# Kinetica-jl/Kinetica.jl

Measured on AMD Instinct MI355X. Metric: RHS evals/sec (batched sweep) + wall-clock per solve_network, 10k-species CRN, higher is better.
Workload: dtype f64; 1 GPU; synthetic CRN 10000 species / 50000 reactions (seed 12345), batched RHS sweep, B=4096 states per GPU with per-state Arrhenius k (500-1200 K); states_per_gpu=4096, parallelism=replicas x1 (no data-path collective)

## Files before the change

include/kinetica_hip.h:

```cpp
#ifndef KINETICA_HIP_H
#define KINETICA_HIP_H

#include <stdint.h>

#ifdef __cplusplus
extern "C" {
#endif

enum {
  KIN_OK = 0,
  KIN_ERR_INVALID_ARG = 1,
  KIN_ERR_UNSUPPORTED = 2,
  KIN_ERR_DEVICE = 3,
  KIN_ERR_SOLVE_FAILED = 4,
  KIN_ERR_CAPACITY = 5,
  KIN_ERR_STATE = 6
};

enum {
  KIN_RETCODE_SUCCESS = 0,
  KIN_RETCODE_MAXITERS = 1,
  KIN_RETCODE_DTLESSTHANMIN = 2,
  KIN_RETCODE_UNSTABLE = 3
};

typedef struct kin_network kin_network;

int kin_network_create(int64_t n_species, int64_t n_reactions,
                       const int64_t* reac_ptr, const int64_t* reac_idx, const int64_t* reac_sto,
                       const int64_t* prod_ptr, const int64_t* prod_idx, const int64_t* prod_sto,
                       int index_base, kin_network** out);
int kin_network_destroy(kin_network* h);
int kin_network_sizes(const kin_network* h, int64_t* n_species, int64_t* n_reactions);
const char* kin_last_error(const kin_network* h);

int kin_set_rates(kin_network* h, const double* k);
int kin_get_rates(kin_network* h, double* k_out);
int kin_set_arrhenius(kin_network* h, const double* Ea, const double* A, double k_max, double t_mult);
int kin_rates_at(kin_network* h, double T, double* k_out);
int kin_arrhenius_eval(const double* Ea, const double* A, int64_t n, double k_max, double t_mult,
                       double T, double* k_out);
int kin_rate_table(kin_network* h, const double* T, int64_t n_stops, double* out_table);

int kin_rhs(kin_network* h, const double* u, double* du);
int kin_rhs_batched(kin_network* h, int64_t B, const double* u, const double* k, double* du);
int kin_rhs_batched_dev(kin_network* h, int64_t B, const double* d_u, const double* d_k, double* d_du, void* stream);

int kin_lib_layout(kin_network* h, int index_base, int64_t* k_len, int64_t* species_of_lib, int64_t* slot_of_reaction,
                   int32_t* species_identity, int64_t* info);
int kin_lib_layout_host(int64_t n_species, int64_t n_reactions, const int64_t* reac_ptr, const int64_t* reac_idx,
                        const int64_t* reac_sto, const int64_t* prod_ptr, const int64_t* prod_idx, const int64_t* prod_sto,
                        int index_base, int hubs, int64_t* info, int64_t* species_of_lib, int64_t* slot_of_reaction,
                        uint64_t* rec, int32_t* rowtab, int32_t* seg_q, int32_t* win_off, int32_t* win_cnt, int32_t* copy_src,
                        int32_t* seg_k);
int kin_lu_analyze_host(int64_t n_species, int64_t n_reactions, const int64_t* reac_ptr, const int64_t* reac_idx,
                        const int64_t* reac_sto, const int64_t* prod_ptr, const int64_t* prod_idx, const int64_t* prod_sto,
                        int index_base, int hub_degree, int max_rounds, int max_tail_degree, int max_degree, int min_round,
                        int64_t* info);
int kin_states_to_lib_dev(kin_network* h, int64_t B, const double* d_in, double* d_out, void* stream);
int kin_states_from_lib_dev(kin_network* h, int64_t B, const double* d_in, double* d_out, void* stream);
int kin_rates_to_lib_dev(kin_network* h, int64_t B, const double* d_k, double* d_k_lib, void* stream);
int kin_rate_table_lib_dev(kin_network* h, const double* T, int64_t n_stops, double* d_out);
int kin_rhs_tiled_dev(kin_network* h, int64_t B, const double* d_u_lib, const double* d_k_lib, const double* d_T,
                      double* d_du_lib, void* stream);
int kin_rhs_batched_T_dev(kin_network* h, int64_t B, const double* d_u, const double* d_T, double* d_du, void* stream);
int kin_rhs_batched_klib_dev(kin_network* h, int64_t B, const double* d_u, const double* d_k_lib, double* d_du, void* stream);

int kin_flux_batched_dev(kin_network* h, int64_t B, const double* d_u, const double* d_k, const int64_t* d_k_row, const double* d_T,
                         const double* d_w, double* d_flux, double* d_rates, void* stream);
int kin_flux_batched(kin_network* h, int64_t B, const double* u, const double* k, int64_t n_k_rows, const int64_t* k_row,
                     const double* T, const double* w, double* flux, double* rates);
int kin_solution_flux(kin_network* h, const double* w, const double* k, int64_t n_k_rows, const int64_t* k_row,
                      const double* T_rows, double* flux, double* rates);

int kin_jac_nnz(kin_network* h, int64_t* nnz);
int kin_jac_pattern(kin_network* h, int64_t* rowptr, int64_t* colidx, int index_base);
int kin_jac_values(kin_network* h, const double* u, double* vals);

typedef struct kin_params {
  double tspan0, tspan1;
  double abstol;
  double reltol;
  int32_t adaptive_tols;
  int32_t update_tols;
  int32_t solve_chunks;
  int32_t ban_negatives;
  double solve_chunkstep;
// ... 79 lines not shown
```

kinetica_jl_amd/capi.py:

```python
from __future__ import annotations

import ctypes
import os
from ctypes import POINTER, c_char_p, c_double, c_int, c_int32, c_int64, c_void_p

import numpy as np

_HERE = os.path.dirname(os.path.abspath(__file__))
LIB_PATH = os.environ.get("KIN_LIB_PATH", os.path.join(_HERE, "libkinetica_hip.so"))

KIN_OK, KIN_ERR_INVALID_ARG, KIN_ERR_UNSUPPORTED, KIN_ERR_DEVICE, KIN_ERR_SOLVE_FAILED, KIN_ERR_CAPACITY, KIN_ERR_STATE = range(7)
RETCODE_NAMES = {0: "Success", 1: "MaxIters", 2: "DtLessThanMin", 3: "Unstable"}

SYMBOLS = [
    "kin_network_create", "kin_network_destroy", "kin_network_sizes", "kin_last_error",
    "kin_set_rates", "kin_get_rates", "kin_set_arrhenius", "kin_rates_at", "kin_arrhenius_eval",
    "kin_rate_table", "kin_rhs", "kin_rhs_batched", "kin_rhs_batched_dev",
    "kin_jac_nnz", "kin_jac_pattern", "kin_jac_values", "kin_solve", "kin_solve_explicit", "kin_solve_continuous", "kin_solution_size",
    "kin_solution_copy", "kin_solution_max", "kin_integrator_init", "kin_integrator_init_continuous", "kin_integrator_step",
    "kin_integrator_state",
    "kin_newton_solve", "kin_device_count", "kin_set_device", "kin_version", "kin_solution_dot", "kin_rate_table_rows",
    "kin_solution_max_dev", "kin_rate_table_dev", "kin_rhs_block_dev",
    "kin_lib_layout", "kin_lib_layout_host", "kin_states_to_lib_dev", "kin_states_from_lib_dev", "kin_rates_to_lib_dev", "kin_rate_table_lib_dev",
    "kin_rhs_tiled_dev", "kin_rhs_batched_T_dev", "kin_rhs_batched_klib_dev", "kin_abi_version", "kin_struct_size",
    "kin_solve_ensemble", "kin_lu_analyze_host", "kin_solve_ensemble_continuous", "kin_solve_ensemble_discrete",
    "kin_resident_probe", "kin_newton_probe", "kin_step_probe",
    "kin_flux_batched", "kin_flux_batched_dev", "kin_solution_flux",
]
ABI_VERSION = 6


STEP_ROWS, STEP_CTRL, STEP_IARGS, STEP_DARGS = 28, 18, 12, 24
STEP_ROW = dict(D=0, y=8, psi=9, d=10, scale=11, f0=12, f1=13, ytmp=14, cs=15, K=16, x=23, out=24, y_new=25, u=26, b=27)
STEP_CTRL_FIELDS = ("dy_norm_old", "dy_norm", "err_norm", "err_m_norm", "err_p_norm", "crate", "scratch0", "scratch1", "scratch2",
                    "scratch3", "newton_done", "converged", "n_iter", "nonfinite", "any_negative", "ticket", "lu_bad", "spec_go")
STEP_OPS = dict(init_D=0, predict=1, accept=2, accept_predict=3, change_D=4, interp=5, norms=6, newton=7, rk_combine=8, rk_error=9, vec=10)
STEP_VEC_OPS = dict(load_u0=0, cs_from_y=1, y_from_cs_clipped=2, y_from_d0=3, ytmp_from_d0=4, ytmp_axpy=5, save_y=6, interp=7)
STEP_IARG_NAMES = ("member", "order", "aux", "copy_out", "go", "iter", "maxit", "publish_always", "crate_from_ctrl", "ban_negatives", "seq")
STEP_DARG_NAMES = ("atol", "rtol", "h", "upd", "tol", "rate_max", "crate0", "tol_first", "dy_first_max", "c", "ts", "t", "h_abs")
STEP_DARG_W = 13


class KinParams(ctypes.Structure):
    _fields_ = [("tspan0", c_double), ("tspan1", c_double), ("abstol", c_double), ("reltol", c_double),
                ("adaptive_tols", c_int32), ("update_tols", c_int32), ("solve_chunks", c_int32),
                ("ban_negatives", c_int32), ("solve_chunkstep", c_double), ("maxiters", c_int64),
                ("save_interval", c_double), ("dtmin", c_double)]


class KinStats(ctypes.Structure):
    _fields_ = [(n, c_int64) for n in ("n_steps", "n_rejected", "n_rhs", "n_jac", "n_factor", "n_linsolve",
                                        "n_newton_fail", "n_chunks", "n_restarts", "n_retries")] + \
               [("final_abstol", c_double), ("final_reltol", c_double), ("wall_seconds", c_double)] + \
               [(n, c_int64) for n in ("lu_dense_dim", "lu_sparse_rows", "lu_rounds", "lu_nnz", "n_lu_reused", "lu_slots", "n_bad_pivot", "n_lu_dropped")]

    def as_dict(self):
        return {n: getattr(self, n) for n, _ in self._fields_}


class KineticaHipError(RuntimeError):
# ... 102 lines not shown


def device_count():
    n = c_int(0)
    lib().kin_device_count(ctypes.byref(n))
    return n.value


def lib_layout_host(net, hubs=0):
    L = lib()
    arrs = [np.ascontiguousarray(a, dtype=np.int64) for a in (net.reac_ptr, net.reac_idx, net.reac_sto, net.prod_ptr,
                                                              net.prod_idx, net.prod_sto)]
    P32, PU64 = POINTER(c_int32), POINTER(ctypes.c_uint64)
    L.kin_lib_layout_host.argtypes = [c_int64, c_int64] + [POINTER(c_int64)] * 6 + [c_int, c_int, POINTER(c_int64), POINTER(c_int64),
                                                                                  POINTER(c_int64), PU64, P32, P32, P32, P32, P32, P32]
    info = np.zeros(10, np.int64)
    head = [int(net.n_species), int(net.n_reactions)] + [_p64(a) for a in arrs] + [0, int(hubs), _p64(info)]
    st = L.kin_lib_layout_host(*head, None, None, None, None, None, None, None, None, None)
    if st != KIN_OK:
        raise KineticaHipError(st, "network has no tiled layout")
    h, T, P, E, n_copy, BS, wbase, Q, k_len, has_singles = [int(x) for x in info]
    sp = np.empty(net.n_species, np.int64); slot = np.empty(net.n_reactions, np.int64)
    rec = np.empty(max(P, 1), np.uint64); rowtab = np.empty(max(2 * Q, 1), np.int32); seg_q = np.empty(T + 1, np.int32)
    woff = np.empty(T, np.int32); wcnt = np.empty(T, np.int32); copy_src = np.empty(max(n_copy, 1), np.int32)
    seg_k = np.empty(2 * T, np.int32)
    i32 = lambda a: a.ctypes.data_as(P32)
    st = L.kin_lib_layout_host(*head, _p64(sp), _p64(slot), rec.ctypes.data_as(PU64), i32(rowtab), i32(seg_q), i32(woff), i32(wcnt),
                               i32(copy_src), i32(seg_k))
    assert st == KIN_OK
    return dict(k_len=k_len, has_singles=bool(has_singles), seg_k=seg_k.reshape(T, 2), h=h, T=T, P=P, E=E, n_copy=n_copy, BS=BS, wbase=wbase, Q=Q, species_of_lib=sp, slot_of_reaction=slot,
                rec=rec[:P], rowtab=rowtab[:2 * Q].reshape(Q, 2), seg_q=seg_q, win_off=woff, win_cnt=wcnt, copy_src=copy_src[:n_copy])


def lu_analyze_host(net, hub_degree=0, max_rounds=0, max_tail_degree=0, max_degree=0, min_round=0):
    L = lib()
    arrs = [np.ascontiguousarray(a, dtype=np.int64) for a in (net.reac_ptr, net.reac_idx, net.reac_sto, net.prod_ptr,
                                                              net.prod_idx, net.prod_sto)]
    L.kin_lu_analyze_host.argtypes = [c_int64, c_int64] + [POINTER(c_int64)] * 6 + [c_int] * 6 + [POINTER(c_int64)]
    info = np.zeros(12, np.int64)
    st = L.kin_lu_analyze_host(int(net.n_species), int(net.n_reactions), *[_p64(a) for a in arrs], 0, int(hub_degree), int(max_rounds),
                               int(max_tail_degree), int(max_degree), int(min_round), _p64(info))
    if st != KIN_OK:
        raise KineticaHipError(st, "symbolic LU analysis failed")
    keys = ("ns", "m", "rounds", "nnzU", "nnzZ", "nnzV", "nnzLZ", "nnzNVU", "w_size", "fused_products", "plan_entries", "plan_tasks")
    return {k: int(v) for k, v in zip(keys, info)}


def arrhenius_eval(Ea, A, T, k_max=None, t_mult=1.0):
    Ea, A = _f64(Ea), _f64(A)
    out = np.empty(len(Ea))
    st = lib().kin_arrhenius_eval(_pd(Ea), _pd(A), len(Ea), float("nan") if k_max is None else k_max, t_mult, T, _pd(out))
    if st != KIN_OK:
        raise KineticaHipError(st, lib().kin_last_error(None).decode())
    return out


class HipNetwork:

    def __init__(self, n_species, reac_ptr, reac_idx, reac_sto, prod_ptr, prod_idx, prod_sto, index_base=0):
        arrs = [np.ascontiguousarray(a, dtype=np.int64) for a in (reac_ptr, reac_idx, reac_sto, prod_ptr, prod_idx, prod_sto)]
        self._h = c_void_p()
        st = lib().kin_network_create(int(n_species), len(arrs[0]) - 1, *[_p64(a) for a in arrs], index_base,
                                      ctypes.byref(self._h))
        if st != KIN_OK:
            raise KineticaHipError(st, lib().kin_last_error(None).decode())
        self.n = int(n_species)
# ... 388 lines not shown
```

kinetica_jl_amd/csrc/network.cpp:

```cpp
#include "network.hpp"

#include <algorithm>
#include <map>
#include <numeric>
#include <string>

namespace kin {

SegPlanHost build_seg_plan(int64_t n_rows, const int32_t* ptr, const int32_t* dst, const int32_t* a,
                           const int32_t* b, const float* c, bool skip_empty, const int32_t* aux,
                           std::vector<int32_t>* slot_of_entry) {
  SegPlanHost P;
  const bool prod = b != nullptr;
  if (slot_of_entry) slot_of_entry->assign((size_t)ptr[n_rows], -1);
  std::vector<int32_t> shorts, longs;
  for (int64_t i = 0; i < n_rows; i++) {
    int32_t len = ptr[i + 1] - ptr[i];
    if (len == 0 && skip_empty) continue;
    (len <= SegPlanHost::SHORT_MAX ? shorts : longs).push_back((int32_t)i);
  }
  {
    std::vector<size_t> start(SegPlanHost::SHORT_MAX + 2, 0);
    for (int32_t r : shorts) start[ptr[r + 1] - ptr[r] + 1]++;
    for (size_t l = 1; l < start.size(); l++) start[l] += start[l - 1];
    std::vector<int32_t> ordered(shorts.size());
    for (int32_t r : shorts) ordered[start[ptr[r + 1] - ptr[r]]++] = r;
    shorts.swap(ordered);
  }
  const size_t n_groups = (shorts.size() + 63) / 64;
  P.grp_off.reserve(n_groups + 1);
  P.grp_off.push_back(0);
  for (size_t g0 = 0; g0 < shorts.size(); g0 += 64) {
    const size_t g1 = std::min(shorts.size(), g0 + 64);
    P.grp_off.push_back(P.grp_off.back() + (ptr[shorts[g1 - 1] + 1] - ptr[shorts[g1 - 1]]));
  }
  {
    const size_t ell = (size_t)P.grp_off.back() * 64;
    if (a) P.ell_a.assign(ell, 0);
    if (b) P.ell_b.assign(ell, prod ? -1 : 0);
    if (!prod) P.ell_c.assign(ell, 0.0f);
// ... 139 lines not shown
      return kq;
    };
    std::map<Key, std::vector<int32_t>> waiting;
    std::vector<int32_t> partner(R, -1);
    std::vector<char> is_plain(R, 0);
    for (int64_t r = 0; r < R; r++) {
      bool plain;
      Key fwd = key_of(r, +1, plain);
      is_plain[r] = plain;
      if (!plain) continue;
      Key rev = key_of(r, -1, plain);
      auto it = waiting.find(rev);
      if (it != waiting.end() && !it->second.empty()) {
        int32_t q = it->second.back(); it->second.pop_back();
        partner[r] = q; partner[q] = (int32_t)r;
      } else waiting[fwd].push_back((int32_t)r);
    }
    for (int64_t r = 0; r < R; r++) {
      if (partner[r] >= 0 && partner[r] < r) continue;
      H.pair_rec.push_back(s16(H.slot_sp[4 * r + 0]) | (s16(H.slot_sp[4 * r + 1]) << 16));
      H.pair_rec.push_back(s16(H.slot_sp[4 * r + 2]) | (s16(H.slot_sp[4 * r + 3]) << 16));
      H.pair_rec.push_back((uint32_t)H.slot_co[r]);
      H.pair_rec.push_back(is_plain[r] ? 0xffffffffu : (s16(H.x0[r]) | (s16(H.x1[r]) << 16)));
      H.pair_k.push_back((int32_t)r);
      H.pair_k.push_back(partner[r]);
    }
    H.pairs_adjacent = (R % 2 == 0) && (H.n_pairs() * 2 == R);
    for (int64_t p = 0; p < H.n_pairs() && H.pairs_adjacent; p++)
      if (H.pair_k[2 * p] != 2 * p || H.pair_k[2 * p + 1] != 2 * p + 1) H.pairs_adjacent = false;
    H.pairs_block = !H.pairs_adjacent && (H.n_pairs() * 2 == R) && R > 0;
    for (int64_t p = 0; p < H.n_pairs() && H.pairs_block; p++)
      if (H.pair_k[2 * p] != p || H.pair_k[2 * p + 1] != H.n_pairs() + p) H.pairs_block = false;
    if ((H.pairs_adjacent || H.pairs_block) && N + 64 <= 16384) {
      bool ok = true;
      std::vector<int32_t> inst((size_t)4 * H.n_pairs());
      for (int64_t p = 0; p < H.n_pairs() && ok; p++) {
        const uint32_t s01 = H.pair_rec[4 * p], s23 = H.pair_rec[4 * p + 1], co = H.pair_rec[4 * p + 2];
        const uint32_t sl[4] = {s01 & 0xffffu, s01 >> 16, s23 & 0xffffu, s23 >> 16};
        uint64_t side[2][2];
        int cnt[2] = {0, 0};
        for (int j = 0; j < 4 && ok; j++) {
          if (sl[j] == 0xffffu) continue;
          const int c = (int)(int8_t)(co >> (8 * j));
          if (c == 0 || c < -2 || c > 2) { ok = false; break; }
          const int sd = c < 0 ? 0 : 1;
          for (int q = 0; q < (c < 0 ? -c : c); q++) {
            if (cnt[sd] >= 2) { ok = false; break; }
            side[sd][cnt[sd]++] = sl[j];
          }
        }
        if (!ok) break;
        const uint64_t dummy = (uint64_t)N + (uint64_t)(p & 63);
        for (int sd = 0; sd < 2; sd++)
          while (cnt[sd] < 2) side[sd][cnt[sd]++] = dummy;
        for (int j = 0; j < 4; j++) inst[4 * p + j] = (int32_t)side[j / 2][j % 2];
      }
      if (ok) {
        const int64_t P = H.n_pairs();
        const int64_t spare = (160 * 1024) / 16 - (N + 64);
        const int K = (int)std::max<int64_t>(0, std::min<int64_t>(32, spare / 7));
        std::vector<int64_t> refs(N, 0);
        for (int64_t q = 0; q < 4 * P; q++) if (inst[q] < N) refs[inst[q]]++;
        std::vector<int32_t> order(N);
        std::iota(order.begin(), order.end(), 0);
        std::stable_sort(order.begin(), order.end(), [&](int32_t x, int32_t y) { return refs[x] > refs[y]; });
        std::vector<int32_t> rank_of(N, -1);
        H.sweep_copy_species.clear();
        for (int r = 0; r < K && r < N && refs[order[r]] >= 64; r++) {
          rank_of[order[r]] = r;
          for (int c = 1; c < 8; c++) H.sweep_copy_species.push_back(order[r]);
        }
        for (int64_t p = 0; p < P; p++) {
          uint64_t f[4];
          for (int j = 0; j < 4; j++) {
            const int32_t sp = inst[4 * p + j];
            const int c = (int)(p & 7);
            f[j] = (sp < N && rank_of[sp] >= 0 && c > 0) ? (uint64_t)(N + 64 + rank_of[sp] * 7 + (c - 1)) : (uint64_t)sp;
          }
          const uint64_t w = f[0] | (f[1] << 14) | (f[2] << 28) | (f[3] << 42);
          H.pair_rec64.push_back((uint32_t)w);
          H.pair_rec64.push_back((uint32_t)(w >> 32));
        }
        for (int64_t p = P; P > 0 && p < P + SWEEP_REC_PAD; p++) {
          const uint64_t d = (uint64_t)N + (uint64_t)(p & 63);
          const uint64_t w = d | (d << 14) | (d << 28) | (d << 42);
          H.pair_rec64.push_back((uint32_t)w);
          H.pair_rec64.push_back((uint32_t)(w >> 32));
        }
      }
    }
    if (!H.pairs_adjacent && !H.pairs_block && (size_t)(N + 64) * 16 <= 160 * 1024) {
      const int64_t P = H.n_pairs();
      for (int64_t p = 0; p < P; p++) {
        const uint32_t s01 = H.pair_rec[4 * p], s23 = H.pair_rec[4 * p + 1], co = H.pair_rec[4 * p + 2], ops = H.pair_rec[4 * p + 3];
        const uint32_t sl[4] = {s01 & 0xffffu, s01 >> 16, s23 & 0xffffu, s23 >> 16};
        const uint32_t dummy = (uint32_t)N + (uint32_t)(p & 63);
        uint32_t side[2][2] = {{dummy, dummy}, {dummy, dummy}};
        int cnt[2] = {0, 0};
        if (ops == 0xffffffffu) {
          for (int j = 0; j < 4; j++) {
            if (sl[j] == 0xffffu) continue;
            const int c = (int)(int8_t)(co >> (8 * j));
            const int sd = c < 0 ? 0 : 1;
            for (int q = 0; q < (c < 0 ? -c : c) && cnt[sd] < 2; q++) side[sd][cnt[sd]++] = sl[j];
          }
        } else {
          H.gen_expl.push_back((int32_t)p);
        }
        H.gen_rec8.push_back(side[0][0] | (side[0][1] << 16));
        H.gen_rec8.push_back(side[1][0] | (side[1][1] << 16));
      }
      H.gen_k = H.pair_k;
// ... 108 lines not shown
```

kinetica_jl_amd/csrc/network.hpp:

```cpp
#pragma once
#include <cstdint>
#include <vector>

#include "common.hpp"

namespace kin {

struct SegPlanHost {
  static constexpr int SHORT_MAX = 8;
  static constexpr int SEG_LEN = 256;
  static constexpr int BLK_PASS = 12288;
  std::vector<int32_t> grp_off;
  std::vector<int32_t> grp_dst;
  std::vector<int32_t> grp_aux;
  std::vector<int32_t> ell_a, ell_b;
  std::vector<float> ell_c;
  std::vector<int32_t> seg_beg, seg_end;
  std::vector<int32_t> seg_dst;
  std::vector<int32_t> seg_aux;
  std::vector<int32_t> blk_beg, blk_end, blk_dst, blk_aux;
  std::vector<int32_t> long_a, long_b;
  std::vector<float> long_c;
  int32_t val_base = -1;
  int32_t ell_total = 0, long_total = 0;
// ... 11 lines not shown
struct NetworkHost {
  int64_t N = 0, R = 0;
  std::vector<int32_t> x0, x1;
  std::vector<int32_t> y0, y1;
  bool products_le2 = true;
  std::vector<int32_t> slot_sp;
  std::vector<int32_t> slot_co;
  std::vector<uint32_t> pair_rec;
  std::vector<int32_t> pair_k;
  std::vector<uint32_t> gen_rec8;
  std::vector<int32_t> gen_k;
  std::vector<int32_t> gen_expl;
  std::vector<int32_t> sweep_copy_species;
  std::vector<uint32_t> pair_rec64;
  int32_t big_H = 0;
  bool big_tail_by_species = false;
  std::vector<int32_t> big_spec_of_label;
  std::vector<uint32_t> big_rec;
  std::vector<uint32_t> big_rec8;
  std::vector<int32_t> big_expl;
  std::vector<int32_t> big_tail_ptr;
  std::vector<uint32_t> big_tail_ent;
  bool pairs_adjacent = false;
  bool pairs_block = false;
  int64_t n_pairs() const { return (int64_t)pair_k.size() / 2; }
  std::vector<int32_t> sp_ptr, sp_rxn;
  std::vector<float> sp_coef;
  std::vector<int32_t> j_ptr, j_col, j_diag;
  std::vector<int32_t> jc_ptr, jc_src;
  std::vector<float> jc_coef;
  int64_t nnz() const { return (int64_t)j_col.size(); }
};

NetworkHost compile_network(int64_t n_species, int64_t n_reactions, const int64_t* reac_ptr,
                            const int64_t* reac_idx, const int64_t* reac_sto, const int64_t* prod_ptr,
                            const int64_t* prod_idx, const int64_t* prod_sto, int index_base);

}
```

kinetica_jl_amd/csrc/tiled.cpp:

```cpp
#include "tiled.hpp"

#include <algorithm>
#include <array>
#include <map>
#include <chrono>
#include <cstdio>
#include <cstdlib>
#include <numeric>

namespace kin {

namespace {

struct UnionFind {
  std::vector<int32_t> par;
  explicit UnionFind(int32_t n) : par(n) { std::iota(par.begin(), par.end(), 0); }
  int32_t find(int32_t x) {
    while (par[x] != x) { par[x] = par[par[x]]; x = par[x]; }
    return x;
  }
  void unite(int32_t a, int32_t b) {
    a = find(a); b = find(b);
    if (a != b) par[b] = a;
  }
};

struct Rec { int32_t f[4]; int32_t kf, kr; };


struct SegCtx {
  const std::vector<Rec>& recs;
  const std::vector<int64_t>& cnt;
  const std::vector<int32_t>& lib_of_species;
// ... 26 lines not shown
  const int32_t n = (int32_t)sorted.size(), h = cx.h;
  Placement pl;
  pl.order = sorted; pl.labs.resize(n); pl.flipped.assign(n, 0);
  for (int32_t i = 0; i < n; i++)
    for (int j = 0; j < 4; j++) {
      uint64_t opt[1 + TILED_COPIES];
      const int no = label_options(cx, sorted[i], j, opt);
      pl.labs[i][j] = no == 0 ? (uint64_t)(h + (i & (TILED_DUMMY - 1))) : opt[no > 1 ? (i & 7) : 0];
    }
  return pl;
}

Placement place_bank_aware(const SegCtx& cx, const std::vector<int32_t>& sorted) {
  const std::vector<Rec>& recs = cx.recs;
  const std::vector<int64_t>& cnt = cx.cnt;
  const int32_t n = (int32_t)sorted.size(), h = cx.h;
  const int SCAN = cx.scan;
  const bool chunked = cx.chunked;
  Placement pl;
  pl.order.resize(n); pl.labs.resize(n); pl.flipped.assign(n, 0);
  std::vector<int32_t>& placed = pl.order;
  std::vector<std::array<uint64_t, 4>>& labs = pl.labs;
  std::vector<char>& flipped = pl.flipped;
  int64_t& sched_slots = pl.slots; int64_t& sched_conflicts = pl.conflicts; int64_t& dbg_defer = pl.deferred;
  auto cls = [&](int32_t p) { return cls_of(recs[p]); };
  auto kind = [&](int32_t p) { return kind_of(cx, recs[p]); };
  auto options = [&](int32_t p, int j, uint64_t* opt) { return label_options(cx, p, j, opt); };
  struct Cand { int32_t p; uint16_t m16[4]; uint32_t m32[4]; int64_t hard; bool sides; int cls; };
  auto make_cand = [&](int32_t p) {
    Cand c{p, {0, 0, 0, 0}, {0, 0, 0, 0}, 0, false, cls(p)};
    for (int j = 0; j < 4; j++) {
      uint64_t opt[1 + TILED_COPIES];
      const int no = options(p, j, opt);
      for (int o = 0; o < no; o++) { c.m16[j] |= (uint16_t)(1u << (opt[o] & 15)); c.m32[j] |= 1u << (opt[o] & 31); }
      if (no > 0) c.hard = std::max(c.hard, cnt[recs[p].f[j]]);
    }
    c.sides = recs[p].kr >= 0 && (recs[p].f[1] >= 0) == (recs[p].f[3] >= 0);
    return c;
  };
  auto sources = [](int o, int* src) {
    const int s0 = (o & 4) ? 2 : 0, s1 = (o & 4) ? 0 : 2;
    src[0] = s0 + (o & 1); src[1] = s0 + ((o & 1) ^ 1);
    src[2] = s1 + ((o >> 1) & 1); src[3] = s1 + (((o >> 1) & 1) ^ 1);
  };
  bool present[8] = {false, false, false, false, false, false, false, false};
  for (int32_t x = 0; x < n; x++) present[kind(sorted[x]) | cls(sorted[x])] = true;
  auto later_home = [&](int x, int c, int kd) {
    for (int c2 = c + 1; c2 < 4; c2++) if (present[kd | c2] && (x & ~c2) == 0) return true;
    return false;
  };
  std::vector<Cand> deferred;
  uint32_t used[4] = {0, 0, 0, 0}, used32[4] = {0, 0, 0, 0};
  int32_t i = 0;
  for (int32_t a = 0; a < n;) {
    int32_t b = a;
    const int c_run = cls(sorted[a]), k_run = kind(sorted[a]);
    while (b < n && cls(sorted[b]) == c_run && kind(sorted[b]) == k_run) b++;
    const bool live[4] = {true, (c_run & 1) != 0, true, (c_run & 2) != 0};
    std::vector<Cand> pool;
    pool.reserve(SCAN + deferred.size());
    for (size_t d = 0; d < deferred.size();)
      if ((deferred[d].cls & ~c_run) == 0 && kind(deferred[d].p) == k_run) { pool.push_back(deferred[d]); deferred[d] = deferred.back(); deferred.pop_back(); }
      else d++;
    int32_t next = a;
    size_t cur = 0;
    for (;;) {
      if (!chunked || pool.empty()) while (pool.size() < (size_t)SCAN && next < b) pool.push_back(make_cand(sorted[next++]));
      if (pool.empty()) break;
      if ((i & 15) == 0) used[0] = used[1] = used[2] = used[3] = 0;
      if ((i & 31) == 0) used32[0] = used32[1] = used32[2] = used32[3] = 0;
      uint32_t fr[4], fr32[4];
      for (int j = 0; j < 4; j++) { fr[j] = ~used[j] & 0xffffu; fr32[j] = ~used32[j]; }
      size_t best = cur % pool.size(); int best_cost = 1 << 20, best_or = 0, fits = 0; int64_t best_hard = -1;
      const int enough = (i & 15) >= 12 ? 1 : 6;
      for (size_t c = 0; c < pool.size() && fits < enough; c++) {
        const size_t q = (cur + c) % pool.size();
        const Cand& k = pool[q];
        if (best_cost <= 4) {
          const bool a0 = ((k.m16[0] | k.m16[1]) & fr[0]) != 0, a2 = ((k.m16[2] | k.m16[3]) & fr[2]) != 0;
          const bool b0 = k.sides && ((k.m16[2] | k.m16[3]) & fr[0]) != 0, b2 = k.sides && ((k.m16[0] | k.m16[1]) & fr[2]) != 0;
          if (!((a0 && a2) || (b0 && b2))) continue;
        }
        auto field_cost = [&](int sj, int j) {
          if (!k.m16[sj]) return (live[j] && !fr[j]) ? 4 : 0;
          if (!(k.m16[sj] & fr[j])) return 4;
          return (k.m32[sj] & fr32[j]) ? 0 : 1;
        };
        int q_cost = 1 << 20;
        for (int sd = 0; sd < (k.sides ? 2 : 1); sd++) {
          const int s0 = sd ? 2 : 0, s1 = sd ? 0 : 2;
          int cr = field_cost(s0, 0) + field_cost(s0 + 1, 1), o_r = 0;
          if (k.m16[s0 + 1] && cr > 0) { const int c2 = field_cost(s0 + 1, 0) + field_cost(s0, 1); if (c2 < cr) { cr = c2; o_r = 1; } }
          int cp = field_cost(s1, 2) + field_cost(s1 + 1, 3), o_p = 0;
          if (k.m16[s1 + 1] && cp > 0) { const int c2 = field_cost(s1 + 1, 2) + field_cost(s1, 3); if (c2 < cp) { cp = c2; o_p = 2; } }
          const int cost = cr + cp;
          q_cost = std::min(q_cost, cost);
          if (cost < best_cost || (cost == best_cost && k.hard > best_hard)) { best_cost = cost; best = q; best_or = o_r | o_p | (sd ? 4 : 0); best_hard = k.hard; }
        }
        fits += q_cost == 0;
      }
      if (best_cost >= 4 && next == b) {
        size_t kept = 0;
        for (size_t q = 0; q < pool.size(); q++)
          if (later_home(pool[q].cls, c_run, k_run)) deferred.push_back(pool[q]); else pool[kept++] = pool[q];
        if (kept < pool.size()) { dbg_defer += pool.size() - kept; pool.resize(kept); cur = 0; continue; }
      }
      const int32_t p = pool[best].p;
      int src[4];
      sources(best_or, src);
      for (int j = 0; j < 4; j++) {
        uint64_t opt[TILED_DUMMY];
        int no = options(p, src[j], opt);
        if (no == 0) {
          if (!live[j]) { labs[i][j] = (uint64_t)(h + (i & (TILED_DUMMY - 1))); continue; }
          for (int d = 0; d < TILED_DUMMY; d++) opt[d] = (uint64_t)(h + ((i + d) & (TILED_DUMMY - 1)));
          no = TILED_DUMMY;
        }
        int pick = -1;
        for (int o = 0; o < no && pick < 0; o++)
          if (!(used[j] >> (opt[o] & 15) & 1u) && !(used32[j] >> (opt[o] & 31) & 1u)) pick = o;
        for (int o = 0; o < no && pick < 0; o++) if (!(used[j] >> (opt[o] & 15) & 1u)) pick = o;
        sched_slots++;
        if (pick < 0) { pick = no > 1 ? i % no : 0; sched_conflicts++; }
        labs[i][j] = opt[pick];
        used[j] |= 1u << (opt[pick] & 15);
        used32[j] |= 1u << (opt[pick] & 31);
      }
      flipped[i] = (best_or & 4) != 0;
      placed[i++] = p;
      pool[best] = pool.back();
      pool.pop_back();
      cur = best + 1;
    }
    a = b;
  }
  return pl;
}

}

TiledHost build_tiled(const NetworkHost& H, int bs, int h_force) {
  TiledHost L;
  const int32_t N = (int32_t)H.N, R = (int32_t)H.R;
  L.N = N; L.R = R; L.BS = bs;
  if (!H.products_le2) { L.why = "a reaction has more than two product molecules"; return L; }
  if (H.N >= (1 << 30)) { L.why = "too many species"; return L; }

  auto key_of = [&](int32_t r, bool reversed) {
    std::array<int32_t, 4> k = {H.x0[r], H.x1[r], H.y0[r], H.y1[r]};
    if (k[1] >= 0 && k[1] < k[0]) std::swap(k[0], k[1]);
    if (k[3] >= 0 && k[3] < k[2]) std::swap(k[2], k[3]);
    if (reversed) { std::swap(k[0], k[2]); std::swap(k[1], k[3]); }
    return k;
  };
  std::vector<Rec> recs;
  recs.reserve((size_t)R / 2 + 16);
  {
    std::map<std::array<int32_t, 4>, std::vector<int32_t>> waiting;
    for (int32_t r = 0; r < R; r++) {
// ... 240 lines not shown
```

kinetica_jl_amd/csrc/tiled_api.cpp:

```cpp
#include "../../include/kinetica_hip.h"

#include <algorithm>
#include <cstdio>
#include <cmath>

#include "handle.hpp"
#include "tiled_kernels.hpp"

using namespace kin;

namespace {

int tiled_block_size(int64_t N) {
  return N <= 2300 ? 256 : (N <= 4850 ? 512 : 1024);
}

void ensure_tiled(kin_network* h) {
  if (!h->tiled_tried) {
    h->tiled_tried = true;
    h->tiled = build_tiled(h->host, tiled_block_size(h->host.N), 0);
    const TiledHost& L = h->tiled;
    if (L.ok) {
      hipStream_t s = h->stream;
      std::vector<int32_t> rxn_of_slot((size_t)L.k_len(), -1);
// ... 78 lines not shown
int kin_lib_layout_host(int64_t n_species, int64_t n_reactions, const int64_t* reac_ptr, const int64_t* reac_idx,
                        const int64_t* reac_sto, const int64_t* prod_ptr, const int64_t* prod_idx, const int64_t* prod_sto,
                        int index_base, int hubs, int64_t* info, int64_t* species_of_lib, int64_t* slot_of_reaction,
                        uint64_t* rec, int32_t* rowtab, int32_t* seg_q, int32_t* win_off, int32_t* win_cnt, int32_t* copy_src,
                        int32_t* seg_k) {
  try {
    const NetworkHost H = compile_network(n_species, n_reactions, reac_ptr, reac_idx, reac_sto, prod_ptr, prod_idx, prod_sto, index_base);
    const TiledHost L = build_tiled(H, tiled_block_size(H.N), hubs);
    if (!L.ok) {
      if (getenv("KIN_TILED_DEBUG")) fprintf(stderr, "[tiled] no layout: %s\n", L.why.c_str());
      return KIN_ERR_UNSUPPORTED;
    }
    if (info) {
      info[0] = L.h; info[1] = L.T; info[2] = L.P; info[3] = L.E; info[4] = L.n_copy; info[5] = L.BS; info[6] = L.wbase;
      info[7] = L.seg_q.back(); info[8] = L.k_len(); info[9] = L.has_singles ? 1 : 0;
    }
    if (species_of_lib) for (int32_t j = 0; j < L.N; j++) species_of_lib[j] = L.species_of_lib[j];
    if (slot_of_reaction) for (int32_t r = 0; r < L.R; r++) slot_of_reaction[r] = L.slot_of_reaction[r];
    if (rec) for (int32_t p = 0; p < L.P; p++) rec[p] = (uint64_t)L.rec[2 * p] | ((uint64_t)L.rec[2 * p + 1] << 32);
    if (rowtab) std::copy(L.rowtab.begin(), L.rowtab.end(), rowtab);
    if (seg_q) std::copy(L.seg_q.begin(), L.seg_q.end(), seg_q);
    if (win_off) std::copy(L.win_off.begin(), L.win_off.end(), win_off);
    if (win_cnt) std::copy(L.win_cnt.begin(), L.win_cnt.end(), win_cnt);
    if (copy_src) std::copy(L.copy_src.begin(), L.copy_src.end(), copy_src);
    if (seg_k) std::copy(L.seg_k.begin(), L.seg_k.end(), seg_k);
  } catch (const KinError& e) {
    return e.code;
  } catch (const std::exception&) {
    return KIN_ERR_INVALID_ARG;
  }
  return KIN_OK;
}

int kin_states_to_lib_dev(kin_network* h, int64_t B, const double* d_in, double* d_out, void* stream) {
  if (!h) return KIN_ERR_INVALID_ARG;
  KIN_TRY(h)
  require(B > 0 && d_in && d_out && d_in != d_out, ERR_INVALID_ARG, "bad arguments");
  ensure_tiled(h);
  states_convert(h, B, true, d_in, d_out, stream ? (hipStream_t)stream : h->stream);
  KIN_CATCH(h)
}

int kin_states_from_lib_dev(kin_network* h, int64_t B, const double* d_in, double* d_out, void* stream) {
  if (!h) return KIN_ERR_INVALID_ARG;
  KIN_TRY(h)
  require(B > 0 && d_in && d_out && d_in != d_out, ERR_INVALID_ARG, "bad arguments");
  ensure_tiled(h);
  states_convert(h, B, false, d_in, d_out, stream ? (hipStream_t)stream : h->stream);
  KIN_CATCH(h)
}

int kin_rates_to_lib_dev(kin_network* h, int64_t B, const double* d_k, double* d_k_lib, void* stream) {
  if (!h) return KIN_ERR_INVALID_ARG;
  KIN_TRY(h)
  require(B > 0 && d_k && d_k_lib && d_k != d_k_lib, ERR_INVALID_ARG, "bad arguments");
  ensure_tiled(h);
  hipStream_t s = stream ? (hipStream_t)stream : h->stream;
  const TiledHost& L = h->tiled;
  if (L.KL == 2 * (int64_t)L.P && h->host.R % 2 == 0 && ((((uintptr_t)d_k) | ((uintptr_t)d_k_lib)) & 15) == 0)
    launch_rates_to_lib_pairs(L.P, h->host.R, B, h->t_kf.p, h->t_kr.p, d_k, d_k_lib, s);
  else
    launch_gather_rows(L.k_len(), h->host.R, B, h->t_rxn_of_slot.p, d_k, d_k_lib, s);
  KIN_CATCH(h)
}

int kin_rate_table_lib_dev(kin_network* h, const double* T, int64_t n_stops, double* d_out) {
// ... 79 lines not shown
```

Baseline: 10.25 million RHS evals/s.

## Place sweep record labels to balance LDS banks across lane groups

Replaces the fixed round-robin assignment of hub copies and dummy slots in the register-resident sweep records with a greedy placer. Within each 16-lane group it picks hub copies, dummy slots and reactant/product side order so that LDS add banks (16) and read banks (32) are spread evenly, with a refinement pass. The aim is fewer bank-conflict serialisation passes in the atomic-add and read phases of the batched RHS kernel. It also adds a host API that reports modelled bank passes, at the cost of more host-side compile time.

```diff
diff --git a/include/kinetica_hip.h b/include/kinetica_hip.h
--- a/include/kinetica_hip.h
+++ b/include/kinetica_hip.h
@@ -53,6 +53,9 @@
                         int index_base, int hubs, int64_t* info, int64_t* species_of_lib, int64_t* slot_of_reaction,
                         uint64_t* rec, int32_t* rowtab, int32_t* seg_q, int32_t* win_off, int32_t* win_cnt, int32_t* copy_src,
                         int32_t* seg_k);
+int kin_sweep_records_host(int64_t n_species, int64_t n_reactions, const int64_t* reac_ptr, const int64_t* reac_idx,
+                           const int64_t* reac_sto, const int64_t* prod_ptr, const int64_t* prod_idx, const int64_t* prod_sto,
+                           int index_base, int64_t* info, uint64_t* rec, int32_t* copy_species, double* passes);
 int kin_lu_analyze_host(int64_t n_species, int64_t n_reactions, const int64_t* reac_ptr, const int64_t* reac_idx,
                         const int64_t* reac_sto, const int64_t* prod_ptr, const int64_t* prod_idx, const int64_t* prod_sto,
                         int index_base, int hub_degree, int max_rounds, int max_tail_degree, int max_degree, int min_round,
diff --git a/kinetica_jl_amd/capi.py b/kinetica_jl_amd/capi.py
--- a/kinetica_jl_amd/capi.py
+++ b/kinetica_jl_amd/capi.py
@@ -25,7 +25,7 @@
     "kin_rhs_tiled_dev", "kin_rhs_batched_T_dev", "kin_rhs_batched_klib_dev", "kin_abi_version", "kin_struct_size",
     "kin_solve_ensemble", "kin_lu_analyze_host", "kin_solve_ensemble_continuous", "kin_solve_ensemble_discrete",
     "kin_resident_probe", "kin_newton_probe", "kin_step_probe",
-    "kin_flux_batched", "kin_flux_batched_dev", "kin_solution_flux",
+    "kin_flux_batched", "kin_flux_batched_dev", "kin_solution_flux", "kin_sweep_records_host",
 ]
 ABI_VERSION = 6
 
@@ -194,6 +194,29 @@
                 rec=rec[:P], rowtab=rowtab[:2 * Q].reshape(Q, 2), seg_q=seg_q, win_off=woff, win_cnt=wcnt, copy_src=copy_src[:n_copy])
 
 
+def sweep_records_host(net):
+    L = lib()
+    arrs = [np.ascontiguousarray(a, dtype=np.int64) for a in (net.reac_ptr, net.reac_idx, net.reac_sto, net.prod_ptr,
+                                                              net.prod_idx, net.prod_sto)]
+    PU64 = POINTER(ctypes.c_uint64)
+    L.kin_sweep_records_host.argtypes = [c_int64, c_int64] + [POINTER(c_int64)] * 6 + [c_int, POINTER(c_int64), PU64, POINTER(c_int32),
+                                                                                     POINTER(c_double)]
+    info = np.zeros(3, np.int64)
+    head = [int(net.n_species), int(net.n_reactions)] + [_p64(a) for a in arrs] + [0, _p64(info)]
+    st = L.kin_sweep_records_host(*head, None, None, None)
+    if st != KIN_OK:
+        raise KineticaHipError(st, "network has no register-resident sweep records")
+    P, n_copy, block = [int(x) for x in info]
+    rec = np.empty(max(P, 1), np.uint64); copy_species = np.empty(max(n_copy, 1), np.int32); passes = np.zeros(4, np.float64)
+    st = L.kin_sweep_records_host(*head, rec.ctypes.data_as(PU64), copy_species.ctypes.data_as(POINTER(c_int32)), _pd(passes))
+    assert st == KIN_OK
+    rec = rec[:P]
+    labels = np.stack([(rec >> np.uint64(14 * j)) & np.uint64(0x3fff) for j in range(4)], axis=1).astype(np.int64)
+    return dict(P=P, rec=rec, labels=labels, copy_species=copy_species[:n_copy], block=bool(block),
+                plain_add_passes=float(passes[0]), plain_read_passes=float(passes[1]),
+                placed_add_passes=float(passes[2]), placed_read_passes=float(passes[3]))
+
+
 def lu_analyze_host(net, hub_degree=0, max_rounds=0, max_tail_degree=0, max_degree=0, min_round=0):
     L = lib()
     arrs = [np.ascontiguousarray(a, dtype=np.int64) for a in (net.reac_ptr, net.reac_idx, net.reac_sto, net.prod_ptr,
diff --git a/kinetica_jl_amd/csrc/lds_banks.hpp b/kinetica_jl_amd/csrc/lds_banks.hpp
--- /dev/null
+++ b/kinetica_jl_amd/csrc/lds_banks.hpp
@@ -0,0 +1,15 @@
+#pragma once
+#include <cstdint>
+
+namespace kin {
+
+constexpr int LDS_ADD_LANES = 16;
+constexpr int LDS_READ_LANES = 32;
+constexpr uint32_t LDS_ADD_BANK_MASK = LDS_ADD_LANES - 1;
+constexpr uint32_t LDS_READ_BANK_MASK = LDS_READ_LANES - 1;
+constexpr uint32_t LDS_ADD_ALL_BANKS = (1u << LDS_ADD_LANES) - 1;
+
+inline int lds_add_bank(uint64_t label) { return (int)(label & LDS_ADD_BANK_MASK); }
+inline int lds_read_bank(uint64_t label) { return (int)(label & LDS_READ_BANK_MASK); }
+
+}
diff --git a/kinetica_jl_amd/csrc/network.cpp b/kinetica_jl_amd/csrc/network.cpp
--- a/kinetica_jl_amd/csrc/network.cpp
+++ b/kinetica_jl_amd/csrc/network.cpp
@@ -1,11 +1,177 @@
 #include "network.hpp"
+#include "lds_banks.hpp"
 
 #include <algorithm>
+#include <cstring>
 #include <map>
 #include <numeric>
 #include <string>
 
+#ifndef KIN_SWEEP_PLACE
+#define KIN_SWEEP_PLACE 1
+#endif
+
 namespace kin {
+
+namespace {
+
+constexpr int SWEEP_DUMMIES = 64, SWEEP_HUB_COPIES = 7;
+
+inline uint64_t sweep_word(const uint32_t* f) { return (uint64_t)f[0] | ((uint64_t)f[1] << 14) | ((uint64_t)f[2] << 28) | ((uint64_t)f[3] << 42); }
+
+std::vector<uint32_t> place_sweep_records(const std::vector<int32_t>& inst, int64_t P, int32_t N, const std::vector<int32_t>& rank_of,
+                                          int n_hubs, bool place) {
+  std::vector<uint32_t> lab((size_t)4 * P);
+  auto hub_entry = [&](int32_t sp, int c) { return c == 0 ? (uint32_t)sp : (uint32_t)(N + SWEEP_DUMMIES + rank_of[sp] * SWEEP_HUB_COPIES + (c - 1)); };
+  if (!place) {
+    for (int64_t p = 0; p < P; p++)
+      for (int j = 0; j < 4; j++) {
+        const int32_t sp = inst[4 * p + j];
+        lab[4 * p + j] = sp >= N ? (uint32_t)(N + (p & (SWEEP_DUMMIES - 1))) : rank_of[sp] >= 0 ? hub_entry(sp, (int)(p & 7)) : (uint32_t)sp;
+      }
+    return lab;
+  }
+  const size_t E = (size_t)N + SWEEP_DUMMIES + (size_t)SWEEP_HUB_COPIES * n_hubs;
+  std::vector<uint16_t> mark_v(4 * E, 0);
+  uint16_t* const mark[4] = {mark_v.data(), mark_v.data() + E, mark_v.data() + 2 * E, mark_v.data() + 3 * E};
+  int cnt_add[4][LDS_ADD_LANES], cnt_read[4][LDS_READ_LANES], fullest[4];
+  auto add = [&](int j, uint32_t l) {
+    fullest[j] = std::max(fullest[j], ++cnt_add[j][lds_add_bank(l)]);
+    cnt_read[j][lds_read_bank(l)]++; mark[j][l]++;
+  };
+  auto take = [&](int j, uint32_t l) {
+    if (cnt_add[j][lds_add_bank(l)]-- == fullest[j]) fullest[j] = *std::max_element(cnt_add[j], cnt_add[j] + LDS_ADD_LANES);
+    cnt_read[j][lds_read_bank(l)]--; mark[j][l]--;
+  };
+  auto cost = [&](int j, uint32_t l, int m) {
+    const int c = cnt_add[j][lds_add_bank(l)];
+    return (mark[j][l] ? 1 << 20 : 0) + (c + 1 > m ? 4096 : 0) + c * 64 + cnt_read[j][lds_read_bank(l)];
+  };
+  auto best_entry = [&](int j, int32_t sp, uint32_t& l) {
+    const int m = fullest[j];
+    if (sp < N && rank_of[sp] < 0) { l = (uint32_t)sp; return cost(j, l, m); }
+    int bc = 1 << 30;
+    if (sp < N) {
+      for (int o = 0; o <= SWEEP_HUB_COPIES; o++) {
+        const uint32_t e = hub_entry(sp, o);
+        const int c = cost(j, e, m);
+        if (c < bc) { bc = c; l = e; }
+      }
+      return bc;
+    }
+    const int least = *std::min_element(cnt_add[j], cnt_add[j] + LDS_ADD_LANES);
+    const int floor = (least + 1 > m ? 4096 : 0) + least * 64;
+    for (int o = 0; o < SWEEP_DUMMIES && bc > floor; o++) {
+      const uint32_t e = (uint32_t)(N + o);
+      if (cnt_add[j][lds_add_bank(e)] != least) continue;
+      const int c = cost(j, e, m);
+      if (c < bc) { bc = c; l = e; }
+    }
+    return bc;
+  };
+  auto put_side = [&](int64_t p, int f0) {
+    const int32_t a = inst[4 * p + f0], b = inst[4 * p + f0 + 1];
+    uint32_t l[2] = {0, 0}, x[2] = {0, 0};
+    int32_t sp[2] = {a, b};
+    const int straight = (a < N ? best_entry(f0, a, l[0]) : 0) + (b < N ? best_entry(f0 + 1, b, l[1]) : 0);
+    if (a != b && straight > 0) {
+      const int crossed = (b < N ? best_entry(f0, b, x[0]) : 0) + (a < N ? best_entry(f0 + 1, a, x[1]) : 0);
+      if (crossed < straight) { std::swap(sp[0], sp[1]); l[0] = x[0]; l[1] = x[1]; }
+    }
+    for (int q = 0; q < 2; q++) {
+      if (sp[q] >= N) best_entry(f0 + q, sp[q], l[q]);
+      lab[4 * p + f0 + q] = l[q];
+      add(f0 + q, l[q]);
+    }
+  };
+  auto alone = [&](int j, uint32_t l) { return cnt_add[j][lds_add_bank(l)] == 1 && cnt_read[j][lds_read_bank(l)] == 1; };
+  auto single_entry = [&](int32_t sp) { return sp < N && rank_of[sp] < 0; };
+  for (int64_t g0 = 0; g0 < P; g0 += LDS_ADD_LANES) {
+    const int64_t g1 = std::min<int64_t>(P, g0 + LDS_ADD_LANES);
+    memset(cnt_add, 0, sizeof cnt_add);
+    memset(fullest, 0, sizeof fullest);
+    if (g0 % LDS_READ_LANES == 0) memset(cnt_read, 0, sizeof cnt_read);
+    for (int64_t p = g1; p < g0 + LDS_ADD_LANES; p++)
+      for (int j = 0; j < 4; j++) add(j, (uint32_t)(N + (p & (SWEEP_DUMMIES - 1))));
+    for (int round = 0; round < 2; round++)
+      for (int64_t p = g0; p < g1; p++)
+        for (int f0 = 0; f0 < 4; f0 += 2)
+          if ((single_entry(inst[4 * p + f0]) || single_entry(inst[4 * p + f0 + 1])) == (round == 0)) put_side(p, f0);
+    for (int64_t p = g0; p < g1; p++)
+      for (int f0 = 0; f0 < 4; f0 += 2) {
+        if (alone(f0, lab[4 * p + f0]) && alone(f0 + 1, lab[4 * p + f0 + 1])) continue;
+        take(f0, lab[4 * p + f0]); take(f0 + 1, lab[4 * p + f0 + 1]);
+        put_side(p, f0);
+      }
+    for (int64_t p = g0; p < g1; p++)
+      for (int j = 0; j < 4; j++) mark[j][lab[4 * p + j]] = 0;
+    for (int64_t p = g1; p < g0 + LDS_ADD_LANES; p++)
+      for (int j = 0; j < 4; j++) mark[j][N + (p & (SWEEP_DUMMIES - 1))] = 0;
+  }
+  return lab;
+}
+
+void sweep_label_passes(const std::vector<uint32_t>& lab, int64_t P, double* add_passes, double* read_passes) {
+  auto passes = [&](int lanes) {
+    int64_t sum = 0, n = 0;
+    for (int64_t g0 = 0; g0 < P; g0 += lanes) {
+      int cnt[4][LDS_READ_LANES];
+      memset(cnt, 0, sizeof cnt);
+      for (int64_t p = g0; p < std::min<int64_t>(P, g0 + lanes); p++)
+        for (int j = 0; j < 4; j++) cnt[j][lab[4 * p + j] & (uint32_t)(lanes - 1)]++;
+      for (int j = 0; j < 4; j++, n++) sum += *std::max_element(cnt[j], cnt[j] + lanes);
+    }
+    return n ? (double)sum / (double)n : 0.0;
+  };
+  *add_passes = passes(LDS_ADD_LANES);
+  *read_passes = passes(LDS_READ_LANES);
+}
+
+bool sweep_instances(const NetworkHost& H, std::vector<int32_t>& inst) {
+  const int64_t N = H.N;
+  inst.resize((size_t)4 * H.n_pairs());
+  for (int64_t p = 0; p < H.n_pairs(); p++) {
+    const uint32_t s01 = H.pair_rec[4 * p], s23 = H.pair_rec[4 * p + 1], co = H.pair_rec[4 * p + 2];
+    const uint32_t sl[4] = {s01 & 0xffffu, s01 >> 16, s23 & 0xffffu, s23 >> 16};
+    uint64_t side[2][2];
+    int cnt[2] = {0, 0};
+    for (int j = 0; j < 4; j++) {
+      if (sl[j] == 0xffffu) continue;
+      const int c = (int)(int8_t)(co >> (8 * j));
+      if (c == 0 || c < -2 || c > 2) return false;
+      const int sd = c < 0 ? 0 : 1;
+      for (int q = 0; q < (c < 0 ? -c : c); q++) {
+        if (cnt[sd] >= 2) return false;
+        side[sd][cnt[sd]++] = sl[j];
+      }
+    }
+    const uint64_t dummy = (uint64_t)N + (uint64_t)(p & 63);
+    for (int sd = 0; sd < 2; sd++)
+      while (cnt[sd] < 2) side[sd][cnt[sd]++] = dummy;
+    for (int j = 0; j < 4; j++) inst[4 * p + j] = (int32_t)side[j / 2][j % 2];
+  }
+  return true;
+}
+
+}
+
+void sweep_model_passes(const NetworkHost& H, double* passes) {
+  std::fill(passes, passes + 4, 0.0);
+  std::vector<int32_t> inst;
+  if (H.pair_rec64.empty() || !sweep_instances(H, inst)) return;
+  const int64_t P = H.n_pairs();
+  std::vector<int32_t> rank_of(H.N, -1);
+  const int n_hubs = (int)H.sweep_copy_species.size() / SWEEP_HUB_COPIES;
+  for (int r = 0; r < n_hubs; r++) rank_of[H.sweep_copy_species[(size_t)r * SWEEP_HUB_COPIES]] = r;
+  const std::vector<uint32_t> plain = place_sweep_records(inst, P, (int32_t)H.N, rank_of, n_hubs, false);
+  std::vector<uint32_t> built((size_t)4 * P);
+  for (int64_t p = 0; p < P; p++) {
+    const uint64_t w = (uint64_t)H.pair_rec64[2 * p] | ((uint64_t)H.pair_rec64[2 * p + 1] << 32);
+    for (int j = 0; j < 4; j++) built[4 * p + j] = (uint32_t)(w >> (14 * j)) & 0x3fffu;
+  }
+  sweep_label_passes(plain, P, &passes[0], &passes[1]);
+  sweep_label_passes(built, P, &passes[2], &passes[3]);
+}
 
 SegPlanHost build_seg_plan(int64_t n_rows, const int32_t* ptr, const int32_t* dst, const int32_t* a,
                            const int32_t* b, const float* c, bool skip_empty, const int32_t* aux,
@@ -211,30 +377,8 @@
     for (int64_t p = 0; p < H.n_pairs() && H.pairs_block; p++)
       if (H.pair_k[2 * p] != p || H.pair_k[2 * p + 1] != H.n_pairs() + p) H.pairs_block = false;
     if ((H.pairs_adjacent || H.pairs_block) && N + 64 <= 16384) {
-      bool ok = true;
-      std::vector<int32_t> inst((size_t)4 * H.n_pairs());
-      for (int64_t p = 0; p < H.n_pairs() && ok; p++) {
-        const uint32_t s01 = H.pair_rec[4 * p], s23 = H.pair_rec[4 * p + 1], co = H.pair_rec[4 * p + 2];
-        const uint32_t sl[4] = {s01 & 0xffffu, s01 >> 16, s23 & 0xffffu, s23 >> 16};
-        uint64_t side[2][2];
-        int cnt[2] = {0, 0};
-        for (int j = 0; j < 4 && ok; j++) {
-          if (sl[j] == 0xffffu) continue;
-          const int c = (int)(int8_t)(co >> (8 * j));
-          if (c == 0 || c < -2 || c > 2) { ok = false; break; }
-          const int sd = c < 0 ? 0 : 1;
-          for (int q = 0; q < (c < 0 ? -c : c); q++) {
-            if (cnt[sd] >= 2) { ok = false; break; }
-            side[sd][cnt[sd]++] = sl[j];
-          }
-        }
-        if (!ok) break;
-        const uint64_t dummy = (uint64_t)N + (uint64_t)(p & 63);
-        for (int sd = 0; sd < 2; sd++)
-          while (cnt[sd] < 2) side[sd][cnt[sd]++] = dummy;
-        for (int j = 0; j < 4; j++) inst[4 * p + j] = (int32_t)side[j / 2][j % 2];
-      }
-      if (ok) {
+      std::vector<int32_t> inst;
+      if (sweep_instances(H, inst)) {
         const int64_t P = H.n_pairs();
         const int64_t spare = (160 * 1024) / 16 - (N + 64);
         const int K = (int)std::max<int64_t>(0, std::min<int64_t>(32, spare / 7));
@@ -249,14 +393,10 @@
           rank_of[order[r]] = r;
           for (int c = 1; c < 8; c++) H.sweep_copy_species.push_back(order[r]);
         }
+        const int n_hubs = (int)H.sweep_copy_species.size() / SWEEP_HUB_COPIES;
+        const std::vector<uint32_t> placed = place_sweep_records(inst, P, (int32_t)N, rank_of, n_hubs, KIN_SWEEP_PLACE != 0);
         for (int64_t p = 0; p < P; p++) {
-          uint64_t f[4];
-          for (int j = 0; j < 4; j++) {
-            const int32_t sp = inst[4 * p + j];
-            const int c = (int)(p & 7);
-            f[j] = (sp < N && rank_of[sp] >= 0 && c > 0) ? (uint64_t)(N + 64 + rank_of[sp] * 7 + (c - 1)) : (uint64_t)sp;
-          }
-          const uint64_t w = f[0] | (f[1] << 14) | (f[2] << 28) | (f[3] << 42);
+          const uint64_t w = sweep_word(&placed[4 * p]);
           H.pair_rec64.push_back((uint32_t)w);
           H.pair_rec64.push_back((uint32_t)(w >> 32));
         }
diff --git a/kinetica_jl_amd/csrc/network.hpp b/kinetica_jl_amd/csrc/network.hpp
--- a/kinetica_jl_amd/csrc/network.hpp
+++ b/kinetica_jl_amd/csrc/network.hpp
@@ -67,6 +67,8 @@
   int64_t nnz() const { return (int64_t)j_col.size(); }
 };
 
+void sweep_model_passes(const NetworkHost& H, double* passes);
+
 NetworkHost compile_network(int64_t n_species, int64_t n_reactions, const int64_t* reac_ptr,
                             const int64_t* reac_idx, const int64_t* reac_sto, const int64_t* prod_ptr,
                             const int64_t* prod_idx, const int64_t* prod_sto, int index_base);
diff --git a/kinetica_jl_amd/csrc/tiled.cpp b/kinetica_jl_amd/csrc/tiled.cpp
--- a/kinetica_jl_amd/csrc/tiled.cpp
+++ b/kinetica_jl_amd/csrc/tiled.cpp
@@ -1,4 +1,5 @@
 #include "tiled.hpp"
+#include "lds_banks.hpp"
 
 #include <algorithm>
 #include <array>
@@ -91,7 +92,7 @@
     for (int j = 0; j < 4; j++) {
       uint64_t opt[1 + TILED_COPIES];
       const int no = options(p, j, opt);
-      for (int o = 0; o < no; o++) { c.m16[j] |= (uint16_t)(1u << (opt[o] & 15)); c.m32[j] |= 1u << (opt[o] & 31); }
+      for (int o = 0; o < no; o++) { c.m16[j] |= (uint16_t)(1u << lds_add_bank(opt[o])); c.m32[j] |= 1u << lds_read_bank(opt[o]); }
       if (no > 0) c.hard = std::max(c.hard, cnt[recs[p].f[j]]);
     }
     c.sides = recs[p].kr >= 0 && (recs[p].f[1] >= 0) == (recs[p].f[3] >= 0);
@@ -126,12 +127,12 @@
     for (;;) {
       if (!chunked || pool.empty()) while (pool.size() < (size_t)SCAN && next < b) pool.push_back(make_cand(sorted[next++]));
       if (pool.empty()) break;
-      if ((i & 15) == 0) used[0] = used[1] = used[2] = used[3] = 0;
-      if ((i & 31) == 0) used32[0] = used32[1] = used32[2] = used32[3] = 0;
+      if ((i & (LDS_ADD_LANES - 1)) == 0) used[0] = used[1] = used[2] = used[3] = 0;
+      if ((i & (LDS_READ_LANES - 1)) == 0) used32[0] = used32[1] = used32[2] = used32[3] = 0;
       uint32_t fr[4], fr32[4];
-      for (int j = 0; j < 4; j++) { fr[j] = ~used[j] & 0xffffu; fr32[j] = ~used32[j]; }
+      for (int j = 0; j < 4; j++) { fr[j] = ~used[j] & LDS_ADD_ALL_BANKS; fr32[j] = ~used32[j]; }
       size_t best = cur % pool.size(); int best_cost = 1 << 20, best_or = 0, fits = 0; int64_t best_hard = -1;
-      const int enough = (i & 15) >= 12 ? 1 : 6;
+      const int enough = (i & (LDS_ADD_LANES - 1)) >= LDS_ADD_LANES - 4 ? 1 : 6;
       for (size_t c = 0; c < pool.size() && fits < enough; c++) {
         const size_t q = (cur + c) % pool.size();
         const Cand& k = pool[q];
@@ -177,13 +178,13 @@
         }
         int pick = -1;
         for (int o = 0; o < no && pick < 0; o++)
-          if (!(used[j] >> (opt[o] & 15) & 1u) && !(used32[j] >> (opt[o] & 31) & 1u)) pick = o;
-        for (int o = 0; o < no && pick < 0; o++) if (!(used[j] >> (opt[o] & 15) & 1u)) pick = o;
+          if (!(used[j] >> lds_add_bank(opt[o]) & 1u) && !(used32[j] >> lds_read_bank(opt[o]) & 1u)) pick = o;
+        for (int o = 0; o < no && pick < 0; o++) if (!(used[j] >> lds_add_bank(opt[o]) & 1u)) pick = o;
         sched_slots++;
         if (pick < 0) { pick = no > 1 ? i % no : 0; sched_conflicts++; }
         labs[i][j] = opt[pick];
-        used[j] |= 1u << (opt[pick] & 15);
-        used32[j] |= 1u << (opt[pick] & 31);
+        used[j] |= 1u << lds_add_bank(opt[pick]);
+        used32[j] |= 1u << lds_read_bank(opt[pick]);
       }
       flipped[i] = (best_or & 4) != 0;
       placed[i++] = p;
diff --git a/kinetica_jl_amd/csrc/tiled_api.cpp b/kinetica_jl_amd/csrc/tiled_api.cpp
--- a/kinetica_jl_amd/csrc/tiled_api.cpp
+++ b/kinetica_jl_amd/csrc/tiled_api.cpp
@@ -134,6 +134,25 @@
   return KIN_OK;
 }
 
+int kin_sweep_records_host(int64_t n_species, int64_t n_reactions, const int64_t* reac_ptr, const int64_t* reac_idx,
+                           const int64_t* reac_sto, const int64_t* prod_ptr, const int64_t* prod_idx, const int64_t* prod_sto,
+                           int index_base, int64_t* info, uint64_t* rec, int32_t* copy_species, double* passes) {
+  try {
+    const NetworkHost H = compile_network(n_species, n_reactions, reac_ptr, reac_idx, reac_sto, prod_ptr, prod_idx, prod_sto, index_base);
+    if (H.pair_rec64.empty()) return KIN_ERR_UNSUPPORTED;
+    const int64_t P = H.n_pairs();
+    if (info) { info[0] = P; info[1] = (int64_t)H.sweep_copy_species.size(); info[2] = H.pairs_block ? 1 : 0; }
+    if (rec) for (int64_t p = 0; p < P; p++) rec[p] = (uint64_t)H.pair_rec64[2 * p] | ((uint64_t)H.pair_rec64[2 * p + 1] << 32);
+    if (copy_species) std::copy(H.sweep_copy_species.begin(), H.sweep_copy_species.end(), copy_species);
+    if (passes) sweep_model_passes(H, passes);
+  } catch (const KinError& e) {
+    return e.code;
+  } catch (const std::exception&) {
+    return KIN_ERR_INVALID_ARG;
+  }
+  return KIN_OK;
+}
+
 int kin_states_to_lib_dev(kin_network* h, int64_t B, const double* d_in, double* d_out, void* stream) {
   if (!h) return KIN_ERR_INVALID_ARG;
   KIN_TRY(h)
```

Result: faster. 10.83 million RHS evals/s, median of 6 (+5.7%).
